# AIR-DISCOVER/TOIST

Hardware: AMD Instinct MI355X
Metric: train images/sec/node (640x640, bs=8/GPU) + matcher index bit-match (higher is better)
Workload: dtype bf16; 1 GPU; configs[1]: ResNet-101 + RoBERTa-base + 6+6 transformer, 100 queries, batch 8/GPU 640x640, 16-token captions, detection loss (labels+boxes+cardinality+contrastive_align, 5 aux layers), dropout 0.1, clip 0.1 + AdamW + EMA (fused HIP tail); random-init weights; every step a different batch (4 resident batches, 0..10 targets per image) through fixed-address inputs; global_batch=8, parallelism=dp1, launch=hipGraph replay, decoder=2 XCD-resident launches (toist_xdec_fwd / toist_xdec_bwd, one image per XCD)

## Files before the change

include/toist_hip.h:

```cpp
#ifndef TOIST_HIP_H
#define TOIST_HIP_H

#include <stddef.h>
#include <stdint.h>

#ifdef __cplusplus
extern "C" {
#endif

#define TOIST_OK 0
#define TOIST_EINVAL (-1)
#define TOIST_EHIP (-2)

#define TOIST_ABI_VERSION 1

#if defined(__GNUC__)
#define TOIST_API __attribute__((visibility("default")))
#else
#define TOIST_API
#endif

TOIST_API int toist_version(void);
TOIST_API int toist_last_error(char* buf, size_t cap);

// ... 367 lines not shown
    int32_t accumulate;
} toist_reduce_desc;
TOIST_API int toist_gemm_effective_split(const toist_gemm* desc);
TOIST_API int toist_splitk_reduce_batch(const toist_reduce_desc* descs, int n, void* stream);

typedef struct toist_conv_pair {
    int32_t M, C;
    int32_t dgrad;
    int32_t lda;
    const void* a;
    const void* w_first;
    const void* w_second;
    const float* shift_mid;
    const float* shift_out;
    const void* res;
    const void* aux_mid;
    const void* aux_out;
    void* mid;
    void* out;
    int32_t ldr, ldaux_mid, ldaux_out, ldmid, ldout, reserved;
} toist_conv_pair;
TOIST_API int toist_conv_pair_bf16(const toist_conv_pair* desc, void* stream);

TOIST_API int toist_opt_chunk_elems(void);
TOIST_API int toist_opt_sqnorm(const toist_opt_tensor* table, const int64_t* grads, const int32_t* chunks, int n_chunks, float* partial, void* stream);
TOIST_API int toist_opt_finish_norm(const float* partial, int n_chunks, float max_norm, float beta1, float beta2, toist_opt_state* state, void* stream);
TOIST_API int toist_opt_finish_norm_guarded(const float* partial, int n_chunks, float max_norm, float beta1, float beta2, toist_opt_state* state,
                        const int32_t* const* veto_i32, int n_veto_i32, const float* const* veto_f32, int n_veto_f32, void* stream);
TOIST_API int toist_opt_adamw_ema(const toist_opt_tensor* table, const int64_t* grads, const int32_t* chunks, int n_chunks,
                        const toist_opt_group* groups, const toist_opt_state* state, float beta1, float beta2, float eps,
                        float ema_decay, void* stream);
TOIST_API int toist_opt_adamw_ema_blocks(const toist_opt_tensor* table, const int64_t* grads, const int32_t* chunks, int n_chunks,
                               const toist_opt_group* groups, const toist_opt_state* state, float beta1, float beta2, float eps,
                               float ema_decay, int max_blocks, void* stream);

TOIST_API int toist_mask_resize_pack(const float* src, int n, int h0, int w0, int max_h, int max_w, int crop_h, int crop_w, int h, int w,
                           float threshold, uint64_t* bits, void* stream);
TOIST_API int toist_mask_resize_pack_batch(const float* src, int batch, int queries, int h0, int w0, int max_h, int max_w, const int64_t* table,
                                 int cap_h, int cap_w, long long capacity_words, float threshold, uint64_t* bits, void* stream);
TOIST_API int toist_mask_pack(const uint8_t* dense, int n, int h, int w, uint64_t* bits, void* stream);
TOIST_API int toist_mask_unpack(const uint64_t* bits, int n, int h, int w, uint8_t* dense, void* stream);
TOIST_API int toist_mask_area(const uint64_t* bits, int n, int h, int w, uint32_t* area, void* stream);
TOIST_API int toist_mask_iou(const uint64_t* dt, int n_dt, const uint64_t* gt, int n_gt, const uint8_t* iscrowd, const uint32_t* area_dt,
                   const uint32_t* area_gt, int h, int w, double* iou, void* stream);
TOIST_API int toist_mask_rle_count(const uint64_t* bits, int n, int h, int w, int32_t* column_transitions, void* stream);
TOIST_API int toist_mask_rle_emit(const uint64_t* bits, int n, int h, int w, const int64_t* column_offset, uint32_t* positions, void* stream);
// ... 24 lines not shown
```

toist_amd/csrc/gemm.hip:

```cpp
#include <cstdlib>
#include <type_traits>

#include "common.h"
#include "gemm_route.h"

namespace toist {


__device__ __forceinline__ float gelu_f(float v) { return 0.5f * v * (1.f + erff(v * 0.70710678118654752f)); }
__device__ __forceinline__ float gelu_grad_f(float a) {
    return 0.5f * (1.f + erff(a * 0.70710678118654752f)) + a * 0.3989422804014327f * __expf(-0.5f * a * a);
}

template <int N, typename F>
__device__ __forceinline__ void static_for(F&& f) {
    if constexpr (N > 0) {
        static_for<N - 1>(f);
        f(std::integral_constant<int, N - 1>{});
    }
}

struct EpiRow {
    long long crow;
    long long rrow;
// ... 2362 lines not shown

__device__ __forceinline__ u32x4_t load16_asm(const i32x4_t& r, const int byte_off) {
    u32x4_t v;
    asm volatile("buffer_load_dwordx4 %0, %1, %2, 0 offen" : "=&v"(v) : "v"(byte_off), "s"(r) : "memory");
    return v;
}
__device__ __forceinline__ u32x2_t load8_asm(const i32x4_t& r, const int byte_off) {
    u32x2_t v;
    asm volatile("buffer_load_dwordx2 %0, %1, %2, 0 offen" : "=&v"(v) : "v"(byte_off), "s"(r) : "memory");
    return v;
}

constexpr int CP_TILE_BYTES = 128 * 64 * 2;
constexpr int CP_STEP_BYTES = 2 * CP_TILE_BYTES;
constexpr int CP_NS = 3;
constexpr int CP_STEPS = 32;
constexpr int CP_A_OFF = 0;
constexpr int CP_MID_OFF = CP_A_OFF + CP_BM * CP_C * 2;
constexpr int CP_RING_OFF = CP_MID_OFF + CP_BM * 128 * 2;
constexpr int CP_SHIFT_OFF = CP_RING_OFF + CP_NS * CP_STEP_BYTES;
constexpr int CP_LDS = CP_SHIFT_OFF + 5 * CP_C * 4;
static_assert(CP_LDS <= 160 * 1024, "conv_pair_kernel: LDS");

template <bool DG, bool SPLIT>
__global__ __launch_bounds__(512, 2) void conv_pair_kernel(const toist_conv_pair p, const float alpha) {
    constexpr int BK = 64, KT = BK * CP_BM;
    constexpr int C = CP_C, C4 = 4 * CP_C;
    extern __shared__ __attribute__((aligned(16))) unsigned char lds_raw[];
    bf16_t* const smem = reinterpret_cast<bf16_t*>(lds_raw);
    const int tid = threadIdx.x, lane = tid & 63, wave = __builtin_amdgcn_readfirstlane(tid >> 6);
    const int g = lane >> 4, c16 = lane & 15;
    const int wm1 = wave >> 2, wn1 = wave & 3;
    const int M = p.M;
    const int nt = (M + CP_BM - 1) / CP_BM, per = (nt + 7) >> 3;
    const int tile_m = (int)(blockIdx.x & 7) * per + (int)(blockIdx.x >> 3);
    if (tile_m >= nt) return;
    const int m0 = tile_m * CP_BM;
    const unsigned lds0 = (unsigned)(size_t)lds_raw;
    const unsigned ring0 = lds0 + CP_RING_OFF;

    float* const sh = reinterpret_cast<float*>(lds_raw + CP_SHIFT_OFF);
    sh[tid] = (!DG && p.shift_mid) ? p.shift_mid[tid] : 0.f;
    sh[tid + 512] = (!DG && p.shift_mid) ? p.shift_mid[tid + 512] : 0.f;
    if (tid < C) sh[C4 + tid] = (!DG && p.shift_out) ? p.shift_out[tid] : 0.f;

    const i32x4_t rsA = make_rsrc(p.a), rsW1 = make_rsrc(p.w_first), rsW2 = make_rsrc(p.w_second), rsMid = make_rsrc(p.mid);
    const i32x4_t rsR = make_rsrc(p.res), rsXm = make_rsrc(DG ? p.aux_mid : p.res), rsXo = make_rsrc(DG ? p.aux_out : p.res);
    constexpr int NR = DG ? 4 : 2;
    auto pcol = [](const int j, const int q) { return 8 * (q >> 2) + 4 * j + (q & 3); };

    int v1[2], v2[2];
#pragma unroll
    for (int it = 0; it < 2; ++it) {
        const int pch = (it * 8 + wave) * 64 + lane;
        if (DG) {
            const int krow = pch >> 4, rc = swz_m<128>(krow, pch & 15);
            v1[it] = (krow * C4 + rc * 8) * 2;
            v2[it] = (krow * C + rc * 8) * 2;
        } else {
            const int row = pch >> 3, kc = swz_k<BK>(row, pch & 7);
            const int prow = (row & ~31) + pcol((row >> 4) & 1, row & 15);
            v1[it] = (prow * C + kc * 8) * 2;
            v2[it] = (row * C4 + kc * 8) * 2;
        }
    }
    auto issue = [&](const int s, const int slot) {
        const int c = s >> 2, q = s & 3;
        const unsigned dst = ring0 + (unsigned)(slot * CP_STEP_BYTES) + (unsigned)wave * 1024u;
#pragma unroll
        for (int tt = 0; tt < 2; ++tt) {
            const unsigned d0 = dst + (unsigned)(tt * CP_TILE_BYTES);
            if (q < 2) {
                const int so = DG ? ((2 * q + tt) * BK * C4 + 128 * c) * 2 : (128 * c * C + (2 * q + tt) * BK) * 2;
                dma16s(d0, rsW1, v1[0], so);
                dma16s(d0 + 8192u, rsW1, v1[1], so);
            } else {
                const int k0 = 128 * c + BK * (q - 2);
                const int so = DG ? (k0 * C + 128 * tt) * 2 : (128 * tt * C4 + k0) * 2;
                dma16s(d0, rsW2, v2[0], so);
                dma16s(d0 + 8192u, rsW2, v2[1], so);
            }
        }
    };

    asm volatile("s_waitcnt vmcnt(0)" ::: "memory");
    {
        const int pa = wave * 64 + lane, ar = pa >> 3, akc = swz_k<BK>(ar, pa & 7);
        const int va = (m0 + ar < M) ? ((m0 + ar) * p.lda + akc * 8) * 2 : OOB;
#pragma unroll
        for (int it = 0; it < 4; ++it) dma16s(lds0 + (unsigned)(CP_A_OFF + it * KT * 2) + (unsigned)wave * 1024u, rsA, va, it * BK * 2);
    }
    issue(0, 0);
    issue(1, 1);

    f32x4_t acc1[2][2];
    f32x4_t acc2[SPLIT ? 2 : 1][4][2];
#pragma unroll
    for (int h = 0; h < (SPLIT ? 2 : 1); ++h)
#pragma unroll
        for (int i = 0; i < 4; ++i)
#pragma unroll
            for (int j = 0; j < 2; ++j) acc2[h][i][j] = f32x4_t{0.f, 0.f, 0.f, 0.f};
    u32x4_t rres[2], raux[2];
    const u32x4_t zero4 = {0u, 0u, 0u, 0u};
    rres[0] = rres[1] = raux[0] = raux[1] = zero4;

    int slot = 0;
    u32x2_t xo[4][2];
    auto step_top = [&](const int s, auto qc) {
        constexpr int q = decltype(qc)::value;
        if (q == 3 && s + 1 == CP_STEPS) wait_vm<(DG ? 10 : 2)>();
        else wait_vm<(q == 0 ? 4 : q == 1 ? 4 + NR : q == 2 ? NR + 6 : 6)>();
        lds_barrier();
    };
    auto refill = [&](const int s) {
        if (s + 2 < CP_STEPS) issue(s + 2, slot >= 1 ? slot - 1 : CP_NS - 1);
// ... 121 lines not shown
        const int m = m0 + i * 16 + c16;
#pragma unroll
        for (int j = 0; j < 2; ++j) {
            const int col = wave * 32 + j * 16 + g * 4;
            f32x4_t a = acc2[0][i][j];
            if (SPLIT) a = a + acc2[SPLIT ? 1 : 0][i][j];
            const f32x4_t sv = *reinterpret_cast<const f32x4_t*>(sh + C4 + col);
            float v[4];
#pragma unroll
            for (int e = 0; e < 4; ++e) v[e] = a[e] * alpha + sv[e];
            if (m < M) {
                if (DG) {
                    const u32x2_t x2 = xo[i][j];
                    v[0] = __uint_as_float(x2[0] << 16) > 0.f ? v[0] : 0.f; v[1] = __uint_as_float(x2[0] & 0xffff0000u) > 0.f ? v[1] : 0.f;
                    v[2] = __uint_as_float(x2[1] << 16) > 0.f ? v[2] : 0.f; v[3] = __uint_as_float(x2[1] & 0xffff0000u) > 0.f ? v[3] : 0.f;
                } else {
#pragma unroll
                    for (int e = 0; e < 4; ++e) v[e] = fmaxf(v[e], 0.f);
                }
                *reinterpret_cast<uint2*>(outp + (size_t)m * p.ldout + col) = make_uint2(pack2bf(v[0], v[1]), pack2bf(v[2], v[3]));
            }
        }
    }
}

static int launch_conv_pair(const toist_conv_pair& d, const bool split, hipStream_t st) {
    const int nt = (d.M + CP_BM - 1) / CP_BM, per = (nt + 7) / 8;
    const dim3 grid(8u * (unsigned)per, 1, 1);
#define TOIST_CONV_PAIR(DG, SP)                                                                                                            \
    do {                                                                                                                                   \
        static std::atomic<unsigned long long> done{0};                                                                                    \
        if (!lds_attr_once_flag(done, [] { return hipFuncSetAttribute((const void*)conv_pair_kernel<DG, SP>, hipFuncAttributeMaxDynamicSharedMemorySize, CP_LDS) == hipSuccess; })) { \
            set_last_error("toist_conv_pair_bf16: cannot enable %d bytes of LDS", CP_LDS);                                                 \
            return TOIST_EHIP;                                                                                                             \
        }                                                                                                                                  \
        hipLaunchKernelGGL((conv_pair_kernel<DG, SP>), grid, dim3(512), CP_LDS, st, d, 1.f);                                               \
    } while (0)
    if (d.dgrad) { if (split) TOIST_CONV_PAIR(true, true); else TOIST_CONV_PAIR(true, false); }
    else { if (split) TOIST_CONV_PAIR(false, true); else TOIST_CONV_PAIR(false, false); }
#undef TOIST_CONV_PAIR
    return TOIST_OK;
}

static int launch_gemm256w(const toist_gemm& d, hipStream_t st) {
    static std::atomic<unsigned long long> done{0};
    if (!lds_attr_once_flag(done, [] {
// ... 379 lines not shown
    if (rc != TOIST_OK || r.post == GEMM_POST_NONE || r.post == GEMM_POST_DEFERRED) return rc;
    if (r.post == GEMM_POST_EPILOGUE) {
        const long long chunks = (long long)d.M * ((d.N + 7) / 8);
        hipLaunchKernelGGL(splitk_epilogue_kernel, dim3((unsigned)((chunks + 255) / 256)), dim3(256), 0, st, d);
        return check_launch("toist_gemm_bf16(splitk epilogue)");
    }
    const long long total4 = ((long long)d.M * d.N) / 4;
    int grid = (int)((total4 + 255) / 256 > 2048 ? 2048 : (total4 + 255) / 256);
    hipLaunchKernelGGL(splitk_reduce_kernel, dim3(grid), dim3(256), 0, st, (const float*)d.workspace, d.split_k, d.M, d.N, d.epi.alpha,
                       d.epi.rscale, d.epi.accumulate, (float*)d.c, d.ldc);
    return check_launch("toist_gemm_bf16(splitk reduce)");
}

extern "C" int toist_conv_pair_bf16(const toist_conv_pair* desc, void* stream) {
    using namespace toist;
    TOIST_REQUIRE(desc != nullptr, "toist_conv_pair_bf16: null descriptor");
    const toist_conv_pair d = *desc;
    const gemm_verdict ok = pair_check(d);
    if (ok.code != TOIST_OK) { set_last_error("%s", ok.msg); return ok.code; }
    const bool split = gemm_route(pair_second_gemm(d)).family == GEMM_128;
    const int rc = launch_conv_pair(d, split, (hipStream_t)stream);
    return rc != TOIST_OK ? rc : check_launch("toist_conv_pair_bf16");
}
#endif
```

toist_amd/csrc/gemm_route.cpp:

```cpp
#include "gemm_route.h"

#include <cstddef>
#include <cstdio>

#include "tuning.h"

namespace toist {

static bool aligned16(const void* p) { return (((size_t)p) & 15) == 0; }

static void normalise(toist_gemm& d) {
    if (d.batch <= 0) d.batch = 1;
    if (d.batch_inner <= 0) d.batch_inner = 1;
    if (d.split_k <= 0) d.split_k = 1;
}

#define GEMM_REQUIRE(v, cond, ...) \
    do { if ((v).code == TOIST_OK && !(cond)) { (v).code = TOIST_EINVAL; std::snprintf((v).msg, sizeof((v).msg), __VA_ARGS__); } } while (0)

gemm_verdict gemm_check(const toist_gemm& desc) {
    gemm_verdict v{};
    toist_gemm d = desc;
    GEMM_REQUIRE(v, d.M > 0 && d.N > 0 && d.K > 0, "toist_gemm_bf16: bad shape M=%d N=%d K=%d", d.M, d.N, d.K);
    normalise(d);
// ... 295 lines not shown
    GEMM_REQUIRE(v, rows * d.lda < lim && rows * d.ldmid < lim && rows * d.ldr < lim && rows * d.ldout < lim &&
                        (!d.dgrad || (rows * d.ldaux_mid < lim && rows * d.ldaux_out < lim)),
                 "toist_conv_pair_bf16: M = %d rows exceed the 2 GiB byte offsets of the kernel", d.M);
    return v;
}

bool pair_applies(const toist_conv_pair& desc) { return pair_check(desc).code == TOIST_OK; }

toist_gemm pair_second_gemm(const toist_conv_pair& p) {
    toist_gemm d{};
    d.M = p.M, d.N = p.C, d.K = 4 * p.C;
    d.a_kind = TOIST_A_ROWK, d.b_kind = p.dgrad ? TOIST_B_KROW : TOIST_B_ROWK;
    d.a.ptr = p.mid, d.a.ld = p.ldmid;
    d.b.ptr = p.w_second, d.b.ld = p.dgrad ? p.C : 4 * p.C;
    d.c = p.out, d.ldc = p.ldout;
    d.batch = d.batch_inner = d.split_k = 1;
    d.epi.alpha = 1.f;
    d.epi.shift = p.shift_out;
    d.epi.act = p.dgrad ? TOIST_ACT_MASK_POS : TOIST_ACT_RELU;
    d.epi.aux = p.aux_out, d.epi.ldaux = p.dgrad ? p.ldaux_out : 0;
    return d;
}

}

extern "C" int toist_gemm_pick_tile(const toist_gemm* desc) { return desc == nullptr ? 0 : toist::gemm_route(*desc).tile; }

extern "C" int toist_gemm_effective_split(const toist_gemm* desc) {
    if (desc == nullptr) return 0;
    toist_gemm d = *desc;
    if (d.workspace == nullptr) d.workspace = (float*)16;
    return toist::gemm_route(d).split;
}
```

toist_amd/csrc/gemm_route.h:

```cpp
#pragma once
#include "../../include/toist_hip.h"

namespace toist {

constexpr int C3_BM = 128, C3_BK = 64, C3_NP = 28;
constexpr int G8_BM = 128, G8_BN = 128, G8_BK = 64;
constexpr int G9_BM = 256, G9_BN = 128, G9_NS = 6;

enum gemm_family {
    GEMM_TILES = 0,
    GEMM_CONV3,
    GEMM_PANEL,
    GEMM_128,
    GEMM_128W,
    GEMM_256W
};

enum gemm_post {
    GEMM_POST_NONE = 0,
    GEMM_POST_REDUCE,
    GEMM_POST_EPILOGUE,
    GEMM_POST_DEFERRED
};

struct gemm_verdict {
    int code;
    char msg[320];
};

struct gemm_plan : gemm_verdict {
    int family;
    int tile;
    int ring;
    int batch, batch_inner, split;
    int post;
};

gemm_verdict gemm_check(const toist_gemm& desc);
gemm_plan gemm_route(const toist_gemm& desc);
bool lean_epilogue_ok(const toist_gemm& d);

constexpr int CP_BM = 64, CP_C = 256;
gemm_verdict pair_check(const toist_conv_pair& desc);
bool pair_applies(const toist_conv_pair& desc);
toist_gemm pair_second_gemm(const toist_conv_pair& desc);

}
```

toist_amd/engine.py:

```python
import math

import weakref

import torch

from . import kernels as k
from . import ops
from .knobs import knob

BF16 = torch.bfloat16


class Var:

    __slots__ = ("data", "grad", "needs_grad", "drop", "gdrop", "plus", "raw_grad")

    def __init__(self, data, needs_grad=True):
        self.data = data
        self.grad = None
        self.needs_grad = needs_grad
        self.raw_grad = False
        self.plus = None
        self.drop = None
        self.gdrop = None
# ... 769 lines not shown
        dqkv = torch.empty(M, 3 * D, dtype=BF16, device=dev)
        k.attn_small_bwd(qkv[:, :D], qkv[:, D:2 * D], qkv[:, 2 * D:], key_pad, B, H, L, dh, scale, p, seed_p, stats, dctx,
                         dqkv[:, :D], dqkv[:, D:2 * D], dqkv[:, 2 * D:], *bias)
        for i, (W, b) in enumerate(proj):
            if W.g is not None:
                tape.linear_wgrad(dqkv[:, i * D:(i + 1) * D], x.data, W, b)
        if x.needs_grad:
            x.grad = ops.linear_dgrad(dqkv, Wpacked, res=x.grad)

    tape.record(bwd)
    return out


def pair_link(w1_next, t1_next):
    return {"w1": w1_next, "t1": t1_next}


def _pair_shapes_ok(a2, w3, w1n, idn):
    C = a2.shape[-1]
    return C == 256 and tuple(w3.shape) == (4 * C, 1, 1, C) and tuple(w1n.shape) == (C, 1, 1, 4 * C) and idn.is_contiguous() \
        and tuple(idn.shape) == (*a2.shape[:3], 4 * C) and a2.is_contiguous()


def bottleneck(tape, x, W, bn, stride, has_down, train, take=None, give=None):
    w1, w2, w3 = krsc(W["conv1"].w), krsc(W["conv2"].w), krsc(W["conv3"].w)
    s1, t1 = bn["bn1"]
    s2, t2 = bn["bn2"]
    s3, t3 = bn["bn3"]
    a1 = take.pop("a1", None) if take is not None else None
    if a1 is None:
        a1 = ops.conv2d(x.data, w1, shift=t1, act=k.ACT_RELU)
    a2 = ops.conv2d(a1, w2, stride=stride, pad=1, shift=t2, act=k.ACT_RELU)
    if has_down:
        wd = krsc(W["down"].w)
        sd, td = bn["down"]
        idn = ops.conv2d(x.data, wd, stride=stride, shift=td)
    else:
        idn = x.data
    w1n = krsc(give["w1"].w) if give is not None else None
    if give is not None and (k.CONV_PAIR & 1) and _pair_shapes_ok(a2, w3, w1n, idn):
        C, M = a2.shape[-1], a2.numel() // a2.shape[-1]
        y = torch.empty(*a2.shape[:3], 4 * C, dtype=BF16, device=a2.device)
        a1n = torch.empty_like(a2)
        k.conv_pair(a2.view(M, C), w3.view(4 * C, C), w1n.view(C, 4 * C), idn.view(M, 4 * C), y.view(M, 4 * C), a1n.view(M, C),
                    shift_mid=t3, shift_out=give["t1"])
        give["a1"] = a1n
    else:
        y = ops.conv2d(a2, w3, shift=t3, res=idn, act=k.ACT_RELU)
    if give is not None and train and (k.CONV_PAIR & 2) and _pair_shapes_ok(a2, w3, w1n, y):
        give["w3"], give["a2"] = w3, a2
    if has_down:
        del idn
    out = Var(y)
    if not train:
        return out
    H, Wd = x.data.shape[1], x.data.shape[2]

    def bwd():
        g3 = out.take_grad()
        stash = give.pop("g", None) if give is not None else None
        if g3 is None:
            return
        tape.conv_wgrad(g3, a2, w3.shape, krsc(W["conv3"].g), s3, view=W["conv3"])
        if stash is not None and stash[0] is g3:
            g2 = stash[1]
        else:
            g2 = ops.conv2d_dgrad(g3, w3, a2.shape[1:3], act=k.ACT_MASK_POS, aux=a2)
        tape.conv_wgrad(g2, a1, w2.shape, krsc(W["conv2"].g), s2, stride=stride, pad=1, view=W["conv2"])
        g1 = ops.conv2d_dgrad(g2, w2, (H, Wd), stride=stride, pad=1, act=k.ACT_MASK_POS, aux=a1)
        tape.conv_wgrad(g1, x.data, w1.shape, krsc(W["conv1"].g), s1, view=W["conv1"])
        if has_down:
            tape.conv_wgrad(g3, x.data, wd.shape, krsc(W["down"].g), sd, stride=stride, view=W["down"])
        if not x.needs_grad:
            return
        prev = x.take_grad()
        if take is not None and "a2" in take and not has_down and prev is None and stride == 1 and g3.is_contiguous():
            C, M = g1.shape[-1], g1.numel() // g1.shape[-1]
            pa2 = take.pop("a2")
            gx, g2p = torch.empty_like(x.data), torch.empty_like(pa2)
            k.conv_pair(g1.view(M, C), w1.view(C, 4 * C), take.pop("w3").view(4 * C, C), g3.view(M, 4 * C), gx.view(M, 4 * C), g2p.view(M, C),
                        dgrad=True, aux_mid=x.data.view(M, 4 * C), aux_out=pa2.view(M, C))
            x.grad = gx
            take["g"] = (gx, g2p)
            return
        if has_down:
            if stride == 1:
                gx = ops.conv2d_dgrad(g3, wd, (H, Wd), res=prev)
            else:
                gx = prev if prev is not None else torch.zeros_like(x.data)
                ops.conv2d_dgrad(g3, wd, (H, Wd), stride=stride, out=gx, res=gx if prev is not None else None)
        else:
            gx = g3
            if prev is not None:
                k.add(prev, g3, prev)
                gx = prev
        x.grad = ops.conv2d_dgrad(g1, w1, (H, Wd), res=gx, act=k.ACT_MASK_POS, aux=x.data)

    tape.record(bwd)
    return out
```

toist_amd/kernels.py:

```python
import ctypes
import os

import torch

from . import _lib
from .folds import FOLDS, _raw_stream
from .knobs import knob
from ._lib import (A_CONV, A_CONVT, A_KROW, A_ROWK, ACT_GELU, ACT_GELU_BWD, ACT_MASK_POS, ACT_NONE, ACT_RELU,
                   ACT_SIGMOID, ACT_SIGMOID_BWD, B_CONVX, B_KROW, B_ROWK, Epilogue, Gemm, Operand)

__all__ = [
    "A_ROWK", "A_KROW", "A_CONV", "A_CONVT", "B_ROWK", "B_KROW", "B_CONVX", "ACT_NONE", "ACT_RELU", "ACT_GELU",
    "ACT_SIGMOID", "ACT_MASK_POS", "ACT_GELU_BWD", "ACT_SIGMOID_BWD", "ConvGeom", "operand", "gemm", "matcher",
    "layernorm_fwd", "layernorm_bwd", "softmax_fwd", "softmax_bwd", "colsum", "add", "dropout", "pack_image", "maxpool3x3s2", "stem_fwd",
    "unpack_nhwc", "sine_position", "embed_fwd", "embed_bwd", "criterion_fwd", "criterion_bwd", "attnmap_softmax_fwd", "attnmap_softmax_bwd",
    "groupnorm_fwd", "groupnorm_apply", "groupnorm_bwd", "upsample_add", "upsample_add_bwd", "sum_queries", "sum_segments", "upsample_add_rows", "mask_stage_fwd", "mask_loss_fwd", "mask_loss_bwd",
]


PROFILE = None
SEED_DEV = None
FORCE_TILE = 0
FORCE_SPLIT = 0
DEBUG_FLAGS = 0
# ... 240 lines not shown

def conv_pair(a, w_first, w_second, res, mid, out, *, dgrad=False, shift_mid=None, shift_out=None, aux_mid=None, aux_out=None):
    M, C = a.shape
    for t in (a, res, mid, out, aux_mid, aux_out):
        if t is not None and (t.dim() != 2 or t.stride(1) != 1 or t.shape[0] != M):
            raise ValueError("conv_pair: operands are [M, width] views with contiguous rows")
    if tuple(w_first.shape) != ((C, 4 * C) if dgrad else (4 * C, C)) or tuple(w_second.shape) != ((4 * C, C) if dgrad else (C, 4 * C)) \
            or not (w_first.is_contiguous() and w_second.is_contiguous()):
        raise ValueError("conv_pair: weights are contiguous [4C, C] / [C, 4C] (forward) or [C, 4C] / [4C, C] (data gradient)")
    if tuple(res.shape) != (M, 4 * C) or tuple(mid.shape) != (M, 4 * C) or tuple(out.shape) != (M, C):
        raise ValueError("conv_pair: res / mid are [M, 4C], out is [M, C]")
    d = ConvPair()
    d.M, d.C, d.dgrad, d.lda = M, C, 1 if dgrad else 0, a.stride(0)
    d.a, d.w_first, d.w_second = _p(a, torch.bfloat16), _p(w_first, torch.bfloat16), _p(w_second, torch.bfloat16)
    d.shift_mid, d.shift_out = _p(shift_mid, torch.float32), _p(shift_out, torch.float32)
    d.res, d.ldr = _p(res, torch.bfloat16), res.stride(0)
    d.aux_mid, d.ldaux_mid = _p(aux_mid, torch.bfloat16), aux_mid.stride(0) if aux_mid is not None else 0
    d.aux_out, d.ldaux_out = _p(aux_out, torch.bfloat16), aux_out.stride(0) if aux_out is not None else 0
    d.mid, d.ldmid, d.out, d.ldout = _p(mid, torch.bfloat16), mid.stride(0), _p(out, torch.bfloat16), out.stride(0)
    CONV_PAIR_CALLS[1 if dgrad else 0] += 1
    _lib.check(_lib.lib().toist_conv_pair_bf16(ctypes.cast(ctypes.pointer(d), ctypes.c_void_p), _stream()), "toist_conv_pair_bf16")


def matcher(logits, boxes, tgt_boxes, pos_map, tgt_off, match_off, max_T, w_class, w_bbox, w_giou, src_idx, tgt_idx,
            status, cost_out=None):
    L, B, Q, K = logits.shape
    _lib.check(
        _lib.lib().toist_matcher(_p(logits, torch.float32), _p(boxes, torch.float32), _p(tgt_boxes, torch.float32),
                                 _p(pos_map, torch.float32), _p(tgt_off, torch.int32), _p(match_off, torch.int32), L, B, Q,
                                 K, max_T, w_class, w_bbox, w_giou, _p(src_idx, torch.int64), _p(tgt_idx, torch.int64),
                                 _p(status, torch.int32), _p(cost_out, torch.float32), _stream()), "toist_matcher")


def layernorm_fwd(x, gamma, beta, eps, y, mean=None, rstd=None, add=None, y2=None):
    rows, D = x.shape
    _lib.check(
        _lib.lib().toist_layernorm_fwd(_p(x, torch.bfloat16), _p(gamma, torch.float32), _p(beta, torch.float32), eps, rows, D,
                                       _p(y, torch.bfloat16), _p(mean, torch.float32), _p(rstd, torch.float32), _p(add, torch.bfloat16),
                                       _p(y2, torch.bfloat16), _stream()),
        "toist_layernorm_fwd")


LN_DEFER = knob("TOIST_LN_DEFER", True)


def _queue_ln_param_grads(blocks, D, dgamma, dbeta):
# ... 664 lines not shown
```

Before: 710.7 images/s.

## Fuse 3x3 bottleneck conv into conv-pair kernel as a chained prologue

Adds a conv_chain kernel that computes the 3x3 stride-1 convolution for a row tile (implicit GEMM over 9 taps, with ReLU or mask epilogue) directly into LDS. It then feeds that tile straight into the existing 1x1 conv pair (conv3 plus the next block's conv1) without a global round trip. It is wired into the forward and data-gradient paths for stride-1 blocks without downsampling. The intent is to remove a kernel launch and the write and read of the intermediate activation. In exchange the kernel uses more LDS and registers, and recomputes halo rows per tile. Default knob value 2 enables only the backward chain.

```diff
diff --git a/include/toist_hip.h b/include/toist_hip.h
--- a/include/toist_hip.h
+++ b/include/toist_hip.h
@@ -413,6 +413,19 @@
 } toist_conv_pair;
 TOIST_API int toist_conv_pair_bf16(const toist_conv_pair* desc, void* stream);
 
+typedef struct toist_conv_chain {
+    toist_conv_pair pair;
+    const void* x;
+    const void* w;
+    const float* shift;
+    const void* mask;
+    int32_t N, H, W;
+    int32_t stride, pad;
+    int32_t ldx, ldmask, reserved;
+} toist_conv_chain;
+TOIST_API int toist_conv_chain_bf16(const toist_conv_chain* desc, void* stream);
+TOIST_API int toist_conv_chain_applies(const toist_conv_chain* desc);
+
 TOIST_API int toist_opt_chunk_elems(void);
 TOIST_API int toist_opt_sqnorm(const toist_opt_tensor* table, const int64_t* grads, const int32_t* chunks, int n_chunks, float* partial, void* stream);
 TOIST_API int toist_opt_finish_norm(const float* partial, int n_chunks, float max_norm, float beta1, float beta2, toist_opt_state* state, void* stream);
diff --git a/toist_amd/csrc/gemm.hip b/toist_amd/csrc/gemm.hip
--- a/toist_amd/csrc/gemm.hip
+++ b/toist_amd/csrc/gemm.hip
@@ -2408,8 +2408,193 @@
 constexpr int CP_LDS = CP_SHIFT_OFF + 5 * CP_C * 4;
 static_assert(CP_LDS <= 160 * 1024, "conv_pair_kernel: LDS");
 
-template <bool DG, bool SPLIT>
-__global__ __launch_bounds__(512, 2) void conv_pair_kernel(const toist_conv_pair p, const float alpha) {
+constexpr int CC_A_BYTES = CP_BM * 64 * 2;
+constexpr int CC_STAGE_BYTES = CC_A_BYTES + CP_C * 64 * 2;
+constexpr int CC_NS = 3;
+constexpr int CC_LDS = CP_LDS + CP_C * 4;
+static_assert(CC_NS * CC_STAGE_BYTES <= CP_SHIFT_OFF && CC_LDS <= 160 * 1024, "conv_chain_kernel: LDS");
+
+template <bool DG, typename Prefetch>
+__device__ __forceinline__ void chain_phase0(const toist_conv_chain& c, const float alpha, const int m0, unsigned char* const lds_raw,
+                                             const float* const sh0, Prefetch&& pair_prefetch) {
+    constexpr int BK = 64, C = CP_C, KT = BK * CP_BM, T = 9 * C / BK, NCH = C / BK, LDB = 9 * C;
+    const int tid = threadIdx.x, lane = tid & 63, wave = __builtin_amdgcn_readfirstlane(tid >> 6);
+    const int kh = wave >> 2, wn = wave & 3, g = lane >> 4, c16 = lane & 15;
+    const int M = c.pair.M, W = c.W, ldx = c.ldx;
+    const unsigned lds0 = (unsigned)(size_t)lds_raw;
+    const i32x4_t rsX = make_rsrc((const bf16_t*)c.x - (long long)(W + 1) * ldx);
+    const i32x4_t rsW = make_rsrc(c.w);
+
+    int va, vb[4];
+    unsigned tapok = 0;
+    {
+        const int pch = wave * 64 + lane, row = pch >> 3, kc = swz_k<BK>(row, pch & 7);
+        const int m = m0 + row, plane = c.H * W;
+        const int mm = m < M ? m : 0;
+        const int rem = mm - (mm / plane) * plane;
+        const int py = rem / W, px = rem - py * W;
+        va = m < M ? (m * ldx + kc * 8) * 2 : OOB;
+#pragma unroll
+        for (int t = 0; t < 9; ++t) {
+            const int iy = py - 1 + t / 3, ix = px - 1 + t % 3;
+            if (iy >= 0 && iy < c.H && ix >= 0 && ix < W) tapok |= 1u << t;
+        }
+    }
+#pragma unroll
+    for (int it = 0; it < 4; ++it) {
+        const int pch = (it * 8 + wave) * 64 + lane, half = pch >> 10, pl = pch & 1023;
+        if (DG) {
+            const int krow = pl >> 4, rc = swz_m<128>(krow, pl & 15);
+            vb[it] = (krow * LDB + half * 128 + rc * 8) * 2;
+        } else {
+            const int row = pl >> 3, kc = swz_k<BK>(row, pl & 7);
+            vb[it] = ((half * 128 + row) * LDB + kc * 8) * 2;
+        }
+    }
+    int i_tap = 0, i_chunk = 0, so_tap = 0;
+    int va_eff = (tapok & 1u) ? va : OOB;
+    auto issue = [&](const int slot) {
+        const unsigned da = lds0 + (unsigned)(slot * CC_STAGE_BYTES) + (unsigned)wave * 1024u, db = da + (unsigned)CC_A_BYTES;
+        const int soa = so_tap + i_chunk * (BK * 2);
+        const int sob = DG ? (i_chunk * BK * LDB + (8 - i_tap) * C) * 2 : (i_tap * NCH + i_chunk) * (BK * 2);
+        unsigned keep;
+        asm volatile("s_mov_b32 %0, m0\n\ts_mov_b32 m0, %1\n\ts_nop 0\n\tbuffer_load_dwordx4 %6, %11, %13 offen lds\n\t"
+                     "s_mov_b32 m0, %2\n\ts_nop 0\n\tbuffer_load_dwordx4 %7, %12, %14 offen lds\n\t"
+                     "s_mov_b32 m0, %3\n\ts_nop 0\n\tbuffer_load_dwordx4 %8, %12, %14 offen lds\n\t"
+                     "s_mov_b32 m0, %4\n\ts_nop 0\n\tbuffer_load_dwordx4 %9, %12, %14 offen lds\n\t"
+                     "s_mov_b32 m0, %5\n\ts_nop 0\n\tbuffer_load_dwordx4 %10, %12, %14 offen lds\n\ts_mov_b32 m0, %0"
+                     : "=&s"(keep)
+                     : "s"(da), "s"(db), "s"(db + 8192u), "s"(db + 16384u), "s"(db + 24576u), "v"(va_eff), "v"(vb[0]), "v"(vb[1]), "v"(vb[2]), "v"(vb[3]),
+                       "s"(rsX), "s"(rsW), "s"(__builtin_amdgcn_readfirstlane(soa)), "s"(__builtin_amdgcn_readfirstlane(sob))
+                     : "memory");
+        if (++i_chunk == NCH) {
+            i_chunk = 0;
+            ++i_tap;
+            so_tap = ((i_tap / 3) * W + i_tap % 3) * ldx * 2;
+            va_eff = ((tapok >> i_tap) & 1u) ? va : OOB;
+        }
+    };
+    issue(0);
+    issue(1);
+
+    const int a_base = (c16 * BK + swz_k<BK>(c16, kh * 4 + g) * 8) * 2;
+    int b_base[4][2];
+#pragma unroll
+    for (int j = 0; j < 4; ++j) {
+        if (DG) {
+            const int k = kh * 32 + 8 * g + (c16 >> 2);
+            const int rc = (((wn & 1) * 64 + j * 16) >> 3) + ((c16 & 3) >> 1), sub = (c16 & 1) * 4;
+            b_base[j][0] = CC_A_BYTES + (wn >> 1) * (BK * 128 * 2) + (k * 128 + swz_m<128>(k, rc) * 8 + sub) * 2;
+            b_base[j][1] = CC_A_BYTES + (wn >> 1) * (BK * 128 * 2) + ((k + 4) * 128 + swz_m<128>(k + 4, rc) * 8 + sub) * 2;
+        } else {
+            const int row = wn * 64 + j * 16 + c16;
+            b_base[j][0] = CC_A_BYTES + (row * BK + swz_k<BK>(row, kh * 4 + g) * 8) * 2;
+            b_base[j][1] = 0;
+        }
+    }
+    f32x4_t acc[4][4];
+#pragma unroll
+    for (int i = 0; i < 4; ++i)
+#pragma unroll
+        for (int j = 0; j < 4; ++j) acc[i][j] = f32x4_t{0.f, 0.f, 0.f, 0.f};
+
+    auto step = [&](auto slotc, const int t) {
+        constexpr int SLOT = decltype(slotc)::value;
+        if (t + 1 < T) wait_vm<5>();
+        else wait_vm<0>();
+        lds_barrier();
+        if (t + 2 < T) issue((SLOT + 2) % CC_NS);
+        bf16x8_t af[4], bfr[4];
+#pragma unroll
+        for (int i = 0; i < 4; ++i) af[i] = *reinterpret_cast<const bf16x8_t*>(lds_raw + a_base + SLOT * CC_STAGE_BYTES + i * 16 * BK * 2);
+#pragma unroll
+        for (int j = 0; j < 4; ++j) {
+            if (DG) {
+                typedef __attribute__((address_space(3))) s16x4_t* lds_v4;
+                union { struct { s16x4_t a, b; } h; bf16x8_t v; } u;
+                u.h.a = __builtin_amdgcn_ds_read_tr16_b64_v4i16((lds_v4)(lds_raw + b_base[j][0] + SLOT * CC_STAGE_BYTES));
+                u.h.b = __builtin_amdgcn_ds_read_tr16_b64_v4i16((lds_v4)(lds_raw + b_base[j][1] + SLOT * CC_STAGE_BYTES));
+                bfr[j] = u.v;
+            } else {
+                bfr[j] = *reinterpret_cast<const bf16x8_t*>(lds_raw + b_base[j][0] + SLOT * CC_STAGE_BYTES);
+            }
+        }
+#pragma unroll
+        for (int i = 0; i < 4; ++i)
+#pragma unroll
+            for (int j = 0; j < 4; ++j) acc[i][j] = __builtin_amdgcn_mfma_f32_16x16x32_bf16(bfr[j], af[i], acc[i][j], 0, 0, 0);
+    };
+    static_assert(T % CC_NS == 0, "conv_chain_kernel: whole trips round the ring");
+#pragma unroll 1
+    for (int t = 0; t < T; t += CC_NS) static_for<CC_NS>([&](auto sc) { step(sc, t + decltype(sc)::value); });
+    lds_barrier();
+
+    const i32x4_t rsO = make_rsrc(c.pair.a), rsK = make_rsrc(DG ? c.mask : c.pair.a);
+    u32x4_t mk[4];
+    if (DG) {
+#pragma unroll
+        for (int it = 0; it < 4; ++it) {
+            const int q = it * 512 + tid, m = m0 + (q >> 5);
+            mk[it] = load16_asm(rsK, m < M ? (m * c.ldmask + (q & 31) * 8) * 2 : OOB);
+        }
+    }
+    pair_prefetch();
+
+    auto xch = [&](const int w) { return reinterpret_cast<float*>(lds_raw + (w < 6 ? w * 8192 : CP_RING_OFF + 2 * CP_STEP_BYTES + (w - 6) * 8192)); };
+    float* const xw = xch(wave);
+#pragma unroll
+    for (int ii = 0; ii < 2; ++ii)
+#pragma unroll
+        for (int j = 0; j < 4; ++j) *reinterpret_cast<f32x4_t*>(xw + ((ii * 4 + j) * 64 + lane) * 4) = kh == 0 ? acc[2 + ii][j] : acc[ii][j];
+    lds_barrier();
+    const float* const xp = xch(wave ^ 4);
+    f32x4_t fin[2][4];
+#pragma unroll
+    for (int ii = 0; ii < 2; ++ii)
+#pragma unroll
+        for (int j = 0; j < 4; ++j) {
+            const f32x4_t o = *reinterpret_cast<const f32x4_t*>(xp + ((ii * 4 + j) * 64 + lane) * 4);
+            fin[ii][j] = (kh == 0 ? acc[ii][j] : acc[2 + ii][j]) + o;
+        }
+    lds_barrier();
+#pragma unroll
+    for (int ii = 0; ii < 2; ++ii) {
+        const int r = (2 * kh + ii) * 16 + c16;
+#pragma unroll
+        for (int j = 0; j < 4; ++j) {
+            const f32x4_t sv = *reinterpret_cast<const f32x4_t*>(sh0 + wn * 64 + j * 16 + g * 4);
+            float v[4];
+#pragma unroll
+            for (int e = 0; e < 4; ++e) v[e] = fin[ii][j][e] * alpha + sv[e];
+            if (!DG) {
+#pragma unroll
+                for (int e = 0; e < 4; ++e) v[e] = fmaxf(v[e], 0.f);
+            }
+            *reinterpret_cast<u32x2_t*>(lds_raw + CP_A_OFF + wn * KT * 2 + (r * BK + swz_k<BK>(r, 2 * j + (g >> 1)) * 8 + (g & 1) * 4) * 2) =
+                u32x2_t{pack2bf(v[0], v[1]), pack2bf(v[2], v[3])};
+        }
+    }
+    lds_barrier();
+    if (DG) asm volatile("s_waitcnt vmcnt(8)" : "+v"(mk[0]), "+v"(mk[1]), "+v"(mk[2]), "+v"(mk[3]) : : "memory");
+#pragma unroll
+    for (int it = 0; it < 4; ++it) {
+        const int q = it * 512 + tid, row = q >> 5, cc = q & 31, m = m0 + row;
+        u32x4_t* const sp = reinterpret_cast<u32x4_t*>(lds_raw + CP_A_OFF + (cc >> 3) * KT * 2 + (row * BK + swz_k<BK>(row, cc & 7) * 8) * 2);
+        u32x4_t o = *sp;
+        if (DG) {
+#pragma unroll
+            for (int e = 0; e < 4; ++e) {
+                const unsigned x = mk[it][e];
+                o[e] = (__uint_as_float(x << 16) > 0.f ? o[e] & 0xffffu : 0u) | (__uint_as_float(x & 0xffff0000u) > 0.f ? o[e] & 0xffff0000u : 0u);
+            }
+            *sp = o;
+        }
+        store16_asm(rsO, m < M ? (m * c.pair.lda + cc * 8) * 2 : OOB, o);
+    }
+}
+
+template <bool DG, bool SPLIT, bool CHAIN>
+__device__ __forceinline__ void conv_pair_body(const toist_conv_pair& p, const float alpha, const toist_conv_chain* const chain) {
     constexpr int BK = 64, KT = BK * CP_BM;
     constexpr int C = CP_C, C4 = 4 * CP_C;
     extern __shared__ __attribute__((aligned(16))) unsigned char lds_raw[];
@@ -2429,6 +2614,7 @@
     sh[tid] = (!DG && p.shift_mid) ? p.shift_mid[tid] : 0.f;
     sh[tid + 512] = (!DG && p.shift_mid) ? p.shift_mid[tid + 512] : 0.f;
     if (tid < C) sh[C4 + tid] = (!DG && p.shift_out) ? p.shift_out[tid] : 0.f;
+    if (CHAIN && tid < C) sh[C4 + C + tid] = (!DG && chain->shift) ? chain->shift[tid] : 0.f;
 
     const i32x4_t rsA = make_rsrc(p.a), rsW1 = make_rsrc(p.w_first), rsW2 = make_rsrc(p.w_second), rsMid = make_rsrc(p.mid);
     const i32x4_t rsR = make_rsrc(p.res), rsXm = make_rsrc(DG ? p.aux_mid : p.res), rsXo = make_rsrc(DG ? p.aux_out : p.res);
@@ -2470,14 +2656,16 @@
     };
 
     asm volatile("s_waitcnt vmcnt(0)" ::: "memory");
-    {
+    if constexpr (CHAIN) {
+        chain_phase0<DG>(*chain, alpha, m0, lds_raw, sh + C4 + C, [&] { issue(0, 0); issue(1, 1); });
+    } else {
         const int pa = wave * 64 + lane, ar = pa >> 3, akc = swz_k<BK>(ar, pa & 7);
         const int va = (m0 + ar < M) ? ((m0 + ar) * p.lda + akc * 8) * 2 : OOB;
 #pragma unroll
         for (int it = 0; it < 4; ++it) dma16s(lds0 + (unsigned)(CP_A_OFF + it * KT * 2) + (unsigned)wave * 1024u, rsA, va, it * BK * 2);
-    }
-    issue(0, 0);
-    issue(1, 1);
+        issue(0, 0);
+        issue(1, 1);
+    }
 
     f32x4_t acc1[2][2];
     f32x4_t acc2[SPLIT ? 2 : 1][4][2];
@@ -2645,6 +2833,34 @@
             }
         }
     }
+}
+
+template <bool DG, bool SPLIT>
+__global__ __launch_bounds__(512, 2) void conv_pair_kernel(const toist_conv_pair p, const float alpha) {
+    conv_pair_body<DG, SPLIT, false>(p, alpha, nullptr);
+}
+
+template <bool DG, bool SPLIT>
+__global__ __launch_bounds__(512, 2) void conv_chain_kernel(const toist_conv_chain c, const float alpha) {
+    conv_pair_body<DG, SPLIT, true>(c.pair, alpha, &c);
+}
+
+static int launch_conv_chain(const toist_conv_chain& d, const bool split, hipStream_t st) {
+    const int nt = (d.pair.M + CP_BM - 1) / CP_BM, per = (nt + 7) / 8;
+    const dim3 grid(8u * (unsigned)per, 1, 1);
+#define TOIST_CONV_CHAIN(DG, SP)                                                                                                           \
+    do {                                                                                                                                   \
+        static std::atomic<unsigned long long> done{0};                                                                                    \
+        if (!lds_attr_once_flag(done, [] { return hipFuncSetAttribute((const void*)conv_chain_kernel<DG, SP>, hipFuncAttributeMaxDynamicSharedMemorySize, CC_LDS) == hipSuccess; })) { \
+            set_last_error("toist_conv_chain_bf16: cannot enable %d bytes of LDS", CC_LDS);                                                \
+            return TOIST_EHIP;                                                                                                             \
+        }                                                                                                                                  \
+        hipLaunchKernelGGL((conv_chain_kernel<DG, SP>), grid, dim3(512), CC_LDS, st, d, 1.f);                                              \
+    } while (0)
+    if (d.pair.dgrad) { if (split) TOIST_CONV_CHAIN(true, true); else TOIST_CONV_CHAIN(true, false); }
+    else { if (split) TOIST_CONV_CHAIN(false, true); else TOIST_CONV_CHAIN(false, false); }
+#undef TOIST_CONV_CHAIN
+    return TOIST_OK;
 }
 
 static int launch_conv_pair(const toist_conv_pair& d, const bool split, hipStream_t st) {
@@ -3070,4 +3286,15 @@
     const int rc = launch_conv_pair(d, split, (hipStream_t)stream);
     return rc != TOIST_OK ? rc : check_launch("toist_conv_pair_bf16");
 }
+
+extern "C" int toist_conv_chain_bf16(const toist_conv_chain* desc, void* stream) {
+    using namespace toist;
+    TOIST_REQUIRE(desc != nullptr, "toist_conv_chain_bf16: null descriptor");
+    const toist_conv_chain d = *desc;
+    const gemm_verdict ok = chain_check(d);
+    if (ok.code != TOIST_OK) { set_last_error("%s", ok.msg); return ok.code; }
+    const bool split = gemm_route(pair_second_gemm(d.pair)).family == GEMM_128;
+    const int rc = launch_conv_chain(d, split, (hipStream_t)stream);
+    return rc != TOIST_OK ? rc : check_launch("toist_conv_chain_bf16");
+}
 #endif
diff --git a/toist_amd/csrc/gemm_route.cpp b/toist_amd/csrc/gemm_route.cpp
--- a/toist_amd/csrc/gemm_route.cpp
+++ b/toist_amd/csrc/gemm_route.cpp
@@ -341,7 +341,58 @@
     return d;
 }
 
-}
+toist_gemm chain_first_gemm(const toist_conv_chain& c) {
+    const toist_conv_pair& p = c.pair;
+    toist_gemm d{};
+    d.M = p.M, d.N = p.C, d.K = 9 * p.C;
+    d.a_kind = p.dgrad ? TOIST_A_CONVT : TOIST_A_CONV, d.b_kind = p.dgrad ? TOIST_B_KROW : TOIST_B_ROWK;
+    d.a.ptr = c.x;
+    d.a.SH = d.a.PH = c.H, d.a.SW = d.a.PW = c.W, d.a.SC = p.C;
+    d.a.R = d.a.S = 3, d.a.stride = c.stride, d.a.pad = c.pad, d.a.dil = 1;
+    d.b.ptr = c.w, d.b.ld = 9 * p.C;
+    if (p.dgrad) d.b.kin = p.C, d.b.tap_stride = p.C;
+    d.c = const_cast<void*>(p.a), d.ldc = p.lda;
+    d.batch = d.batch_inner = d.split_k = 1;
+    d.epi.alpha = 1.f;
+    d.epi.shift = c.shift;
+    d.epi.act = p.dgrad ? TOIST_ACT_MASK_POS : TOIST_ACT_RELU;
+    d.epi.aux = c.mask, d.epi.ldaux = p.dgrad ? c.ldmask : 0;
+    return d;
+}
+
+gemm_verdict chain_check(const toist_conv_chain& c) {
+    const toist_conv_pair& p = c.pair;
+    gemm_verdict v{};
+    const long long lim = 1ll << 30;
+    GEMM_REQUIRE(v, c.N > 0 && c.H > 0 && c.W > 0 && (long long)c.N * c.H * c.W == p.M, "toist_conv_chain_bf16: bad shape N=%d H=%d W=%d for M=%d rows",
+                 c.N, c.H, c.W, p.M);
+    GEMM_REQUIRE(v, c.stride == 1 && c.pad == 1, "toist_conv_chain_bf16: stride = %d pad = %d (3x3, stride 1, pad 1 only)", c.stride, c.pad);
+    GEMM_REQUIRE(v, c.x && c.w, "toist_conv_chain_bf16: null operand");
+    if (p.dgrad) {
+        GEMM_REQUIRE(v, c.mask != nullptr, "toist_conv_chain_bf16: the data gradient needs mask");
+        GEMM_REQUIRE(v, c.shift == nullptr, "toist_conv_chain_bf16: the data gradient takes no shift");
+    } else {
+        GEMM_REQUIRE(v, c.mask == nullptr, "toist_conv_chain_bf16: mask belongs to the data gradient (dgrad = 1)");
+    }
+    GEMM_REQUIRE(v, aligned16(c.x) && aligned16(c.w) && aligned16(c.shift) && aligned16(c.mask), "toist_conv_chain_bf16: every pointer must be 16-byte aligned");
+    GEMM_REQUIRE(v, c.ldx >= CP_C && (c.ldx % 8) == 0 && (!p.dgrad || (c.ldmask >= CP_C && (c.ldmask % 8) == 0)),
+                 "toist_conv_chain_bf16: leading dimensions must cover the row and be multiples of 8 (ldx=%d ldmask=%d)", c.ldx, c.ldmask);
+    if (v.code != TOIST_OK) return v;
+    const gemm_verdict pv = pair_check(p);
+    if (pv.code != TOIST_OK) return pv;
+    const long long rows = (long long)((p.M + CP_BM - 1) / CP_BM) * CP_BM + 2ll * c.W + 2;
+    GEMM_REQUIRE(v, rows * c.ldx + CP_C < lim && (!p.dgrad || rows * c.ldmask < lim), "toist_conv_chain_bf16: M = %d rows exceed the 2 GiB byte offsets of the kernel", p.M);
+    const gemm_plan first = gemm_route(chain_first_gemm(c));
+    GEMM_REQUIRE(v, first.code == TOIST_OK && first.family == GEMM_128,
+                 "toist_conv_chain_bf16: at M = %d the 3x3 product does not run on the 128x128 kernel (tile %d), whose sums the chain reproduces", p.M, first.tile);
+    return v;
+}
+
+bool chain_applies(const toist_conv_chain& desc) { return chain_check(desc).code == TOIST_OK; }
+
+}
+
+extern "C" int toist_conv_chain_applies(const toist_conv_chain* desc) { return desc != nullptr && toist::chain_applies(*desc) ? 1 : 0; }
 
 extern "C" int toist_gemm_pick_tile(const toist_gemm* desc) { return desc == nullptr ? 0 : toist::gemm_route(*desc).tile; }
 
diff --git a/toist_amd/csrc/gemm_route.h b/toist_amd/csrc/gemm_route.h
--- a/toist_amd/csrc/gemm_route.h
+++ b/toist_amd/csrc/gemm_route.h
@@ -45,4 +45,8 @@
 bool pair_applies(const toist_conv_pair& desc);
 toist_gemm pair_second_gemm(const toist_conv_pair& desc);
 
+gemm_verdict chain_check(const toist_conv_chain& desc);
+bool chain_applies(const toist_conv_chain& desc);
+toist_gemm chain_first_gemm(const toist_conv_chain& desc);
+
 }
diff --git a/toist_amd/engine.py b/toist_amd/engine.py
--- a/toist_amd/engine.py
+++ b/toist_amd/engine.py
@@ -815,6 +815,23 @@
         and tuple(idn.shape) == (*a2.shape[:3], 4 * C) and a2.is_contiguous()
 
 
+def _chain_shapes_ok(src, w2, w3, w1n, wide):
+    C = src.shape[-1]
+    return src.is_contiguous() and tuple(w2.shape) == (C, 3, 3, C) and _pair_shapes_ok(src, w3, w1n, wide)
+
+
+def _chain_forward(a1, w2, t2, w3, t3, w1n, t1n, idn):
+    if not _chain_shapes_ok(a1, w2, w3, w1n, idn):
+        return None
+    C, M = a1.shape[-1], a1.numel() // a1.shape[-1]
+    a2, a1n = torch.empty_like(a1), torch.empty_like(a1)
+    y = torch.empty(*a1.shape[:3], 4 * C, dtype=BF16, device=a1.device)
+    if not k.conv_chain(a1, w2, a2.view(M, C), w3.view(4 * C, C), w1n.view(C, 4 * C), idn.view(M, 4 * C), y.view(M, 4 * C), a1n.view(M, C),
+                        shift=t2, shift_mid=t3, shift_out=t1n, if_applies=True):
+        return None
+    return a2, y, a1n
+
+
 def bottleneck(tape, x, W, bn, stride, has_down, train, take=None, give=None):
     w1, w2, w3 = krsc(W["conv1"].w), krsc(W["conv2"].w), krsc(W["conv3"].w)
     s1, t1 = bn["bn1"]
@@ -823,27 +840,32 @@
     a1 = take.pop("a1", None) if take is not None else None
     if a1 is None:
         a1 = ops.conv2d(x.data, w1, shift=t1, act=k.ACT_RELU)
-    a2 = ops.conv2d(a1, w2, stride=stride, pad=1, shift=t2, act=k.ACT_RELU)
-    if has_down:
-        wd = krsc(W["down"].w)
-        sd, td = bn["down"]
-        idn = ops.conv2d(x.data, wd, stride=stride, shift=td)
+    w1n = krsc(give["w1"].w) if give is not None else None
+    chained = None
+    if give is not None and (k.CONV_PAIR & k.CONV_CHAIN & 1) and stride == 1 and not has_down:
+        chained = _chain_forward(a1, w2, t2, w3, t3, w1n, give["t1"], x.data)
+    if chained is not None:
+        a2, y, give["a1"] = chained
     else:
-        idn = x.data
-    w1n = krsc(give["w1"].w) if give is not None else None
-    if give is not None and (k.CONV_PAIR & 1) and _pair_shapes_ok(a2, w3, w1n, idn):
-        C, M = a2.shape[-1], a2.numel() // a2.shape[-1]
-        y = torch.empty(*a2.shape[:3], 4 * C, dtype=BF16, device=a2.device)
-        a1n = torch.empty_like(a2)
-        k.conv_pair(a2.view(M, C), w3.view(4 * C, C), w1n.view(C, 4 * C), idn.view(M, 4 * C), y.view(M, 4 * C), a1n.view(M, C),
-                    shift_mid=t3, shift_out=give["t1"])
-        give["a1"] = a1n
-    else:
-        y = ops.conv2d(a2, w3, shift=t3, res=idn, act=k.ACT_RELU)
+        a2 = ops.conv2d(a1, w2, stride=stride, pad=1, shift=t2, act=k.ACT_RELU)
+        if has_down:
+            wd = krsc(W["down"].w)
+            sd, td = bn["down"]
+            idn = ops.conv2d(x.data, wd, stride=stride, shift=td)
+        else:
+            idn = x.data
+        if give is not None and (k.CONV_PAIR & 1) and _pair_shapes_ok(a2, w3, w1n, idn):
+            C, M = a2.shape[-1], a2.numel() // a2.shape[-1]
+            y = torch.empty(*a2.shape[:3], 4 * C, dtype=BF16, device=a2.device)
+            a1n = torch.empty_like(a2)
+            k.conv_pair(a2.view(M, C), w3.view(4 * C, C), w1n.view(C, 4 * C), idn.view(M, 4 * C), y.view(M, 4 * C), a1n.view(M, C),
+                        shift_mid=t3, shift_out=give["t1"])
+            give["a1"] = a1n
+        else:
+            y = ops.conv2d(a2, w3, shift=t3, res=idn, act=k.ACT_RELU)
+        del idn
     if give is not None and train and (k.CONV_PAIR & 2) and _pair_shapes_ok(a2, w3, w1n, y):
         give["w3"], give["a2"] = w3, a2
-    if has_down:
-        del idn
     out = Var(y)
     if not train:
         return out
@@ -860,19 +882,31 @@
         else:
             g2 = ops.conv2d_dgrad(g3, w3, a2.shape[1:3], act=k.ACT_MASK_POS, aux=a2)
         tape.conv_wgrad(g2, a1, w2.shape, krsc(W["conv2"].g), s2, stride=stride, pad=1, view=W["conv2"])
-        g1 = ops.conv2d_dgrad(g2, w2, (H, Wd), stride=stride, pad=1, act=k.ACT_MASK_POS, aux=a1)
+        plain = x.needs_grad and take is not None and "a2" in take and not has_down and x.grad is None and stride == 1 and g3.is_contiguous()
+        g1 = None
+        if plain:
+            C, M = a1.shape[-1], a1.numel() // a1.shape[-1]
+            pa2, pw3 = take.pop("a2"), take.pop("w3")
+            gx, g2p = torch.empty_like(x.data), torch.empty_like(pa2)
+            if (k.CONV_CHAIN & 2) and g2.is_contiguous() and _chain_shapes_ok(a1, w2, pw3, w1, x.data):
+                g1 = torch.empty_like(a1)
+                if not k.conv_chain(g2, w2, g1.view(M, C), w1.view(C, 4 * C), pw3.view(4 * C, C), g3.view(M, 4 * C), gx.view(M, 4 * C),
+                                    g2p.view(M, C), dgrad=True, mask=a1.view(M, C), aux_mid=x.data.view(M, 4 * C), aux_out=pa2.view(M, C),
+                                    if_applies=True):
+                    g1 = None
+        chained = g1 is not None
+        if not chained:
+            g1 = ops.conv2d_dgrad(g2, w2, (H, Wd), stride=stride, pad=1, act=k.ACT_MASK_POS, aux=a1)
         tape.conv_wgrad(g1, x.data, w1.shape, krsc(W["conv1"].g), s1, view=W["conv1"])
         if has_down:
             tape.conv_wgrad(g3, x.data, wd.shape, krsc(W["down"].g), sd, stride=stride, view=W["down"])
         if not x.needs_grad:
             return
         prev = x.take_grad()
-        if take is not None and "a2" in take and not has_down and prev is None and stride == 1 and g3.is_contiguous():
-            C, M = g1.shape[-1], g1.numel() // g1.shape[-1]
-            pa2 = take.pop("a2")
-            gx, g2p = torch.empty_like(x.data), torch.empty_like(pa2)
-            k.conv_pair(g1.view(M, C), w1.view(C, 4 * C), take.pop("w3").view(4 * C, C), g3.view(M, 4 * C), gx.view(M, 4 * C), g2p.view(M, C),
-                        dgrad=True, aux_mid=x.data.view(M, 4 * C), aux_out=pa2.view(M, C))
+        if plain:
+            if not chained:
+                k.conv_pair(g1.view(M, C), w1.view(C, 4 * C), pw3.view(4 * C, C), g3.view(M, 4 * C), gx.view(M, 4 * C), g2p.view(M, C),
+                            dgrad=True, aux_mid=x.data.view(M, 4 * C), aux_out=pa2.view(M, C))
             x.grad = gx
             take["g"] = (gx, g2p)
             return
diff --git a/toist_amd/kernels.py b/toist_amd/kernels.py
--- a/toist_amd/kernels.py
+++ b/toist_amd/kernels.py
@@ -286,6 +286,56 @@
     _lib.check(_lib.lib().toist_conv_pair_bf16(ctypes.cast(ctypes.pointer(d), ctypes.c_void_p), _stream()), "toist_conv_pair_bf16")
 
 
+class ConvChain(ctypes.Structure):
+    _fields_ = [("pair", ConvPair)] + [(n, ctypes.c_void_p) for n in ("x", "w", "shift", "mask")] + \
+               [(n, ctypes.c_int32) for n in ("N", "H", "W", "stride", "pad", "ldx", "ldmask", "reserved")]
+
+
+CONV_CHAIN = knob("TOIST_CONV_CHAIN", 2)
+CONV_CHAIN_CALLS = [0, 0]
+
+
+def _chain_desc(x, w, a, w_first, w_second, res, mid, out, dgrad, shift, mask, shift_mid, shift_out, aux_mid, aux_out):
+    N, H, W, C = x.shape
+    M = N * H * W
+    if x.stride(3) != 1 or x.stride(2) < C or x.stride(1) != W * x.stride(2) or x.stride(0) != H * x.stride(1):
+        raise ValueError("conv_chain: x is [N, H, W, C] with one pixel stride")
+    for t in (a, res, mid, out, aux_mid, aux_out, mask):
+        if t is not None and (t.dim() != 2 or t.stride(1) != 1 or t.shape[0] != M):
+            raise ValueError("conv_chain: operands are [M, width] views with contiguous rows")
+    if tuple(w.shape) != (C, 3, 3, C) or not w.is_contiguous():
+        raise ValueError("conv_chain: w is contiguous [C, 3, 3, C]")
+    if tuple(w_first.shape) != ((C, 4 * C) if dgrad else (4 * C, C)) or tuple(w_second.shape) != ((4 * C, C) if dgrad else (C, 4 * C)) \
+            or not (w_first.is_contiguous() and w_second.is_contiguous()):
+        raise ValueError("conv_chain: weights are contiguous [4C, C] / [C, 4C] (forward) or [C, 4C] / [4C, C] (data gradient)")
+    if tuple(a.shape) != (M, C) or tuple(res.shape) != (M, 4 * C) or tuple(mid.shape) != (M, 4 * C) or tuple(out.shape) != (M, C):
+        raise ValueError("conv_chain: a / out are [M, C], res / mid are [M, 4C]")
+    d = ConvChain()
+    p = d.pair
+    p.M, p.C, p.dgrad, p.lda = M, C, 1 if dgrad else 0, a.stride(0)
+    p.a, p.w_first, p.w_second = _p(a, torch.bfloat16), _p(w_first, torch.bfloat16), _p(w_second, torch.bfloat16)
+    p.shift_mid, p.shift_out = _p(shift_mid, torch.float32), _p(shift_out, torch.float32)
+    p.res, p.ldr = _p(res, torch.bfloat16), res.stride(0)
+    p.aux_mid, p.ldaux_mid = _p(aux_mid, torch.bfloat16), aux_mid.stride(0) if aux_mid is not None else 0
+    p.aux_out, p.ldaux_out = _p(aux_out, torch.bfloat16), aux_out.stride(0) if aux_out is not None else 0
+    p.mid, p.ldmid, p.out, p.ldout = _p(mid, torch.bfloat16), mid.stride(0), _p(out, torch.bfloat16), out.stride(0)
+    d.x, d.w, d.shift = _p(x, torch.bfloat16), _p(w, torch.bfloat16), _p(shift, torch.float32)
+    d.mask, d.ldmask = _p(mask, torch.bfloat16), mask.stride(0) if mask is not None else 0
+    d.N, d.H, d.W, d.stride, d.pad, d.ldx = N, H, W, 1, 1, x.stride(2)
+    return d
+
+
+def conv_chain(x, w, a, w_first, w_second, res, mid, out, *, dgrad=False, shift=None, mask=None, shift_mid=None, shift_out=None, aux_mid=None,
+               aux_out=None, if_applies=False):
+    d = _chain_desc(x, w, a, w_first, w_second, res, mid, out, dgrad, shift, mask, shift_mid, shift_out, aux_mid, aux_out)
+    ref = ctypes.cast(ctypes.pointer(d), ctypes.c_void_p)
+    if if_applies and not _lib.lib().toist_conv_chain_applies(ref):
+        return False
+    CONV_CHAIN_CALLS[1 if dgrad else 0] += 1
+    _lib.check(_lib.lib().toist_conv_chain_bf16(ref, _stream()), "toist_conv_chain_bf16")
+    return True
+
+
 def matcher(logits, boxes, tgt_boxes, pos_map, tgt_off, match_off, max_T, w_class, w_bbox, w_giou, src_idx, tgt_idx,
             status, cost_out=None):
     L, B, Q, K = logits.shape
```

Result: no change. 716.3 images/s (median of 6 runs) (+0.8%).
